# WonderfulToolchain/psxavenc

Hardware: AMD Instinct MI355X
Metric: bs_v2_320x240_frames_per_sec (higher is better)
Workload: dtype int32

## Files before the change

psxavenc_amd/csrc/mdec_kernels.hip:

```cpp

#include <hip/hip_runtime.h>
#include <stdint.h>
#include <type_traits>
#include <stdlib.h>
#include <string.h>

#include "bs_vlc_lut.h"
#include "mdec_search.h"
#include "psxhip_internal.h"
#include "wave_ops.h"

namespace {

constexpr int kWavesSmall = 12, kOccSmall = 6;
constexpr int kWavesLarge = 16, kOccLarge = 4;
constexpr int kTileStride = 72;
constexpr int kZStride = 64;
constexpr int kPilotMax = 4;
constexpr int kMaxTiles = 16;
constexpr uint32_t kNoMb = 0xFFFFu;
constexpr uint32_t kRetryEmpty = 0xFFFFFFFFu, kRetryAbandoned = 0xFFFFFFFEu;
constexpr int kQueueWord = 64;
constexpr int kStartedWord = 96;
constexpr int kLeaveWord = 8;
// ... 926 lines not shown
            phi = *(const uint2*)(frame + o_hi);
        };
        auto fetch = [&](int fx, int fy) { fetch_at((uint32_t)fy * (uint32_t)(8 * W), (uint32_t)fx * 16u); };
        auto mb_bytes = [&](const uint4& ts, uint32_t& b_lo, uint32_t& b_hi) {
            b_lo = __builtin_amdgcn_perm(plo.y, plo.x, ts.x);
            b_hi = __builtin_amdgcn_perm(phi.y, phi.x, ts.y);
        };
        auto fetch_behind = [&](uint32_t row, uint32_t col, uint32_t& b_lo, uint32_t& b_hi) {
            asm volatile("" : "+v"(b_lo), "+v"(b_hi));
            const uint4 tp = L.tab_pix[lane];
            uint32_t o_lo = tp.x + (row << tp.z) + col;
            asm volatile("" : "+v"(o_lo) : "v"(b_lo), "v"(b_hi));
            const uint32_t o_hi = o_lo + tp.y;
            plo = *(const uint2*)(frame + o_lo);
            phi = *(const uint2*)(frame + o_hi);
        };
        auto dct_mb = [&](const uint4& ts, uint32_t b_lo, uint32_t b_hi) {
            int d[8];
            u32x16 ck;
            asm volatile("s_load_dwordx16 %0, %1, %2" : "=s"(ck) : "s"(__builtin_amdgcn_kernarg_segment_ptr()), "n"(offsetof(FrameJob, col_k)));
            {
                fdct8_rows_mfma(b_lo, b_hi, make_uint2(ts.z, ts.w), d);
                const int n = lane & 31;
                int16_t* t0 = tileT + (n >> 3) * kTileStride + (n & 7) + (lane >> 5) * 32;
                store_row_outputs(t0, d);
                if (n < 16) store_row_outputs(t0 + 4 * kTileStride, d + 4);
            }
            wave_sync();
            if (lane < 48) {
                uint4 q;
                asm volatile("ds_read2_b64 %0, %2 offset1:1\n\ts_waitcnt lgkmcnt(0)"
                             : "=v"(q), "+s"(ck) : "v"((uint32_t)(uintptr_t)&tileT[blk * kTileStride + r8 * 8]) : "memory");
                fdct8_col_acc_k(q.x, q.y, __builtin_amdgcn_alignbit(q.w, q.w, 16), __builtin_amdgcn_alignbit(q.z, q.z, 16), ck, d);
                if (r8 == 0) d[0] = CODEC == 0 ? (int)((uint32_t)quant_dc(d[0] >> 17) << 17) : 0;
                uint4 o;
                o.x = pack_sh17(d[1], d[0]);
                o.y = pack_sh17(d[3], d[2]);
                o.z = pack_sh17(d[5], d[4]);
                o.w = pack_sh17(d[7], d[6]);
                *(uint4*)&tileZ[lane * 8] = o;
            }
            wave_sync();
        };

        if (tid == 0) {
            int hint = L.scalars[S_HINT];
            int hint_budget = L.scalars[S_HINT_BUDGET];
            bool local = hint >= 1 && L.scalars[S_HINT_FRAME] == f - 1;
            if (hint < 1) {
                const int sh = L.scalars[S_SHARED_HINT];
                hint = sh & 0xFF;
                hint_budget = sh >> 8;
            }
            const int retry_scale = L.scalars[S_RETRY];
            if (retry_scale > 0) {
                hint = retry_scale;
                hint_budget = max_size;
                local = true;
            }
            const bool hint_ok = hint >= 1 && hint <= 63 && hint_budget == max_size;
            const int dts = L.scalars[S_DISTRUST];
            const int rp = L.scalars[S_REPILOT];
            const int trust_mode = PSX_JOB_INT(trust_mode);
            const bool distrust = trust_mode == 0 ? ((dts & 1) != 0 || (dts >> 8) >= 2) : trust_mode == 2;
            const bool trust_hint = hint_ok && (local || !distrust) && rp == 0;
            L.scalars[S_ABORTS_LEFT] = rp ? 1 : 2;
            L.scalars[S_FOREIGN] = hint_ok && !local ? hint : 0;
// ... 18 lines not shown
                st.fail = (uint64_t)(uint32_t)z | ((uint64_t)(uint32_t)in_loop(0) << 32);
                st.fs[0] = st.fs[1] = st.fb[0] = st.fb[1] = z;
                st.gs[0] = st.gs[1] = st.gb[0] = st.gb[1] = z;
            }
        };
        unsigned long long trace = 0;
        int n_pass = 0, first_abort = 0, guess0 = 0;
        int guess;
        MdecSearch* srch = (MdecSearch*)&L.scalars[S_SEARCH];
        group_sync(1);
        if (L.scalars[S_PILOT_GUESS] == 0) {
        float cfp[kPilotPerWave][6];
#pragma unroll
        for (int i = 0; i < kPilotPerWave; i++) {
            const int pi = wid + i * kWavesPerGroup;
            if (pi < n_pilot) {
                const unsigned u = (unsigned)(2 * pi + 1);
                const int p_fy = (int)((u * (unsigned)ny) / (unsigned)(2 * n_pilot));
                const int p_fx = (int)((((u * 40503u) >> 1) & 0xFFFFu) * (unsigned)nx >> 16);
                fetch(n_pilot == nmb ? pi % nx : p_fx, n_pilot == nmb ? pi / nx : p_fy);
                {
                    const uint4 ts = L.tab_sel[lane];
                    uint32_t b_lo, b_hi;
                    mb_bytes(ts, b_lo, b_hi);
                    dct_mb(ts, b_lo, b_hi);
                }
#pragma unroll
                for (int b = 0; b < 6; b++) cf[b] = lane == 0 ? 0.0f : (float)(int)tileZ[b * kZStride + lc.zsrc];
                wave_sync();
            }
#pragma unroll
            for (int b = 0; b < 6; b++) cfp[i][b] = pi < n_pilot ? cf[b] : 0.0f;
        }
        if (tid == 0) {
            L.scalars[S_PILOTED] = 1;
            const int h0 = L.scalars[S_PILOT_HI];
            MdecSearch st;
            search_reset(st);
            *srch = st;
            const MdecPilot pl = mdec_pilot_next(st, h0, limit_bits, fixed_bits, 0);
            L.scalars[S_PILOT_N] = pl.n;
            L.scalars[S_PILOT_SCALE0 + 0] = pl.s[0];
            L.scalars[S_PILOT_SCALE0 + 1] = pl.s[1];
            L.scalars[S_PILOT_SCALE0 + 2] = pl.s[2];
            L.scalars[S_PILOT_LO] = in_loop(0);
        }
        for (;;) {
            group_sync(1);
            const int np = L.scalars[S_PILOT_N];
            if (np == 0) break;
            if (wid < n_pilot) {
                for (int j = 0; j < np; j++) {
                    const int s = L.scalars[S_PILOT_SCALE0 + j];
                    const QuantK k = make_quant(lc.quant, s);
                    int acc = 0;
#pragma unroll
                    for (int i = 0; i < kPilotPerWave; i++)
                        if (i < pilot_rounds) acc += count_mb(cfp[i], k, lc, L.ac_len16) & 0xFF;
                    const int t = wave::reduce_add(acc);
                    if (lane == 0) atomicAdd(&L.scalars[S_PILOT_BITS0 + j], t);
                }
            }
            group_sync(1);
            if (tid == 0) {
                MdecSearch st = *srch;
                for (int j = 0; j < np; j++) {
                    const int s = L.scalars[S_PILOT_SCALE0 + j];
                    const int est = (int)((long long)L.scalars[S_PILOT_BITS0 + j] * nmb / n_pilot) + fixed_bits;
                    mdec_search_note(st, s, est, est, limit_bits);
                    L.scalars[S_PILOT_BITS0 + j] = 0;
                }
                *srch = st;
                const int round = L.scalars[S_PILOT_LO] + 1;
                const MdecPilot pl = mdec_pilot_next(st, L.scalars[S_PILOT_HI], limit_bits, fixed_bits, round);
                L.scalars[S_PILOT_N] = pl.n;
                L.scalars[S_PILOT_LO] = round;
                L.scalars[S_PILOT_SCALE0 + 0] = pl.s[0];
                L.scalars[S_PILOT_SCALE0 + 1] = pl.s[1];
                L.scalars[S_PILOT_SCALE0 + 2] = pl.s[2];
                if (pl.n == 0) L.scalars[S_PILOT_GUESS] = pl.guess;
            }
        }
        }
        guess = L.scalars[S_PILOT_GUESS];
        if (STATS) { guess0 = carry_pass ? carry_guess0 : guess; if (carry_pass) first_abort = carry_abort; }
        mark(2);

        if (tid == 0) {
            L.scalars[S_NEXT_DRAW] = (int)next_draw;
            MdecSearch st;
            search_reset(st);
            MdecPass np;
            if (limit_bits < fixed_bits || bad_budget) {
                np.done = 1; np.count_scale = 0; np.emit_scale = 0;
            } else {
                np = mdec_search_next(st, guess, limit_bits, fixed_bits);
            }
            *srch = st;
            L.scalars[S_PASS_COUNT] = np.count_scale;
            L.scalars[S_PASS_EMIT] = np.emit_scale;
            L.scalars[S_DONE] = np.done;
            L.scalars[S_RESULT] = st.best;
            L.scalars[S_MB_NEXT] = 2 * kWavesPerGroup;
        }
        group_sync(1);

        while (!L.scalars[S_DONE]) {
            const int count_scale = L.scalars[S_PASS_COUNT], emit_scale = L.scalars[S_PASS_EMIT];
            n_pass++;
            if (STATS && n_pass <= 4) trace |= (unsigned long long)(emit_scale ? emit_scale : count_scale | 0x40) << (24 + 8 * n_pass);
            if (emit_scale && n_pass > 1) {
                for (int i = tid; i < job.stg_words; i += kThreads) L.stg[i] = 0u;
                if (tid == 0) L.scalars[S_STG_NEXT] = 0;
                group_sync(5);
            }
            typedef const char __attribute__((address_space(4))) * OrderBytes;
            typedef const uint32_t __attribute__((address_space(4))) * OrderPtr;
            const OrderBytes order_b = (OrderBytes)(uintptr_t)job.order;
            const int n_tickets = job.trips * kWavesPerGroup;
            auto order_at = [&](int t) -> uint2 {
                const uint32_t byte = min((uint32_t)t, (uint32_t)n_tickets) * 8u;
                const OrderPtr e = (OrderPtr)(order_b + byte);
                return make_uint2(e[0], e[1]);
            };
            int cur_t = wid, nxt_t = wid + kWavesPerGroup;
            uint2 cur_o = order_at(cur_t);
            uint2 nxt_o = order_at(nxt_t);
            fetch_at(cur_o.x & 0x7FFFFFFFu, cur_o.y & 0xFFFFu);
            const QuantK kc = make_quant(lc.quant, count_scale ? count_scale : 1);
            const QuantK ke = make_quant(lc.quant, emit_scale ? emit_scale : 1);
            int acc_cnt = 0;
            int acc_edef = 0;
            int n_codes = 0;
            int emit_bits = 0, mb_done = 0;
            int prev_len = 0;
            const uint32_t thr_low = (uint32_t)((lc.quant * (count_scale ? count_scale : 1) + 1) >> 1);
            const uint32_t thr_emit = (uint32_t)((lc.quant * (emit_scale ? emit_scale : 1) + 1) >> 1);
            const uint32_t thr_list = count_scale ? thr_low : thr_emit;
            const uint32_t low_off = thr_list - 1u, low_span = lane == 0 ? 0u : 2u * thr_list - 1u;
            const uint32_t emit_off = thr_emit - 1u, emit_span = lane == 0 ? 0u : 2u * thr_emit - 1u;
            auto flush = [&]() {
                if (count_scale) {
                    const int tf = wave::reduce_add(acc_cnt & 0xFFFF), td = wave::reduce_add((int)((unsigned)acc_cnt >> 16));
                    if (lane == 0) { atomicAdd(&L.scalars[S_CNT_F], tf); atomicAdd(&L.scalars[S_CNT_D], td); }
                    acc_cnt = 0;
                }
                if (emit_scale) {
                    const int td = wave::reduce_add(acc_edef), tc = n_codes;
                    if (lane == 0) {
                        atomicAdd(&L.scalars[S_EMIT_BITS], emit_bits);
                        atomicAdd(&L.scalars[S_EMIT_D], td);
                        atomicAdd(&L.scalars[S_NNZ], tc - 6 * mb_done);
                    }
                    acc_edef = 0; n_codes = 0; emit_bits = 0;
                }
                if (lane == 0) atomicAdd(&L.scalars[S_CK_DONE], mb_done);
                mb_done = 0;
            };
            const int check_t = (job.trips >= 8 && L.scalars[S_ABORTS_LEFT] > 0) ? (job.trips >> 2) * kWavesPerGroup : n_tickets;
            bool aborted = false, checked = false;

            for (int it = 0; cur_t < n_tickets; it++) {
                if (!checked && cur_t >= check_t) {
                    checked = true;
                    flush();
                    int arrived = 0;
                    if (lane == 0) arrived = atomicAdd(&L.scalars[S_CK_WAVES], 1);
                    const bool judge = __builtin_amdgcn_readfirstlane(arrived) == kWavesPerGroup - 1;
                    unsigned ck_s1 = 0, ck_sq = 0;
                    bool records_ok = false;
                    if (judge && emit_scale) records_ok = __hip_atomic_load(&L.scalars[S_STG_NEXT], __ATOMIC_RELAXED, __HIP_MEMORY_SCOPE_WORKGROUP) <= job.stg_words;
                    if (records_ok) {
                        for (int t = lane; t < check_t; t += 64) {
                            const OrderPtr oe = (OrderPtr)(order_b + (uint32_t)t * 8u);
                            if ((int)oe[0] < 0) {
                                const unsigned x = *(const uint32_t*)((const char*)L.rec + (oe[1] >> 16)) >> 18;
                                ck_s1 += x;
                                ck_sq += x * x;
                            }
                        }
                        ck_s1 = (unsigned)wave::reduce_add((int)ck_s1);
                        ck_sq = (unsigned)wave::reduce_add((int)ck_sq);
                    }
                    if (judge && lane == 0) {
                        const int done = L.scalars[S_CK_DONE];
                        long long pa = 0, pb = 0;
                        if (count_scale) pa = (long long)L.scalars[S_CNT_F] * nmb / done + fixed_bits;
                        if (emit_scale) pb = (long long)L.scalars[S_EMIT_BITS] * nmb / done + 10;
                        int margin = (limit_bits - fixed_bits) / 50;
                        if (emit_scale && records_ok && done > 1 && done < nmb) {
                            const float n = (float)done, mean = (float)ck_s1 / n;
                            float var = (float)ck_sq / n - mean * mean;
                            var = var > 0.0f ? var : 0.0f;
                            const float se = 4.0f * __builtin_sqrtf(var * n * (1.0f - n / (float)nmb)) * ((float)nmb / n);
                            margin = (int)(se * kCkMargin * 0.001f);
                        }
                        int g = mdec_search_checkpoint_bits(*srch, count_scale, (int)pa, emit_scale, (int)pb, limit_bits, fixed_bits, margin);
                        {
                            const int cur = emit_scale ? emit_scale : count_scale + 1, far = cur > 8 ? cur >> 2 : 2;
                            if (g && L.scalars[S_PILOTED] && (g - cur >= far || cur - g >= far)) {
                                const bool too_low = emit_scale && pb > (long long)limit_bits + 4 * margin;
                                const bool too_high = count_scale && pa <= (long long)limit_bits - 4 * margin;
                                if (!too_low && !too_high) g = 0;
                            }
                        }
                        if (g) {
                            L.scalars[S_ABORT] = g | (n_pass << 8);
                            L.scalars[S_ABORTS_LEFT] = L.scalars[S_ABORTS_LEFT] - 1;
                            atomicMax(&L.scalars[S_MB_NEXT], 0x40000000);
                        }
                    }
                }
                if (WAVES == kWavesSmall) {
                    asm volatile("s_bitcmp1_b32 %0, %1\n\ts_cbranch_scc1 1f\n\ts_setprio 0\n\ts_branch 2f\n1:\ts_setprio 1\n2:" : : "s"(prio_bits4), "s"(it) : "scc");
                }
                int drawn = 0;
                if (lane == 0) drawn = atomicAdd(&L.scalars[S_MB_NEXT], 1);
                const bool valid = (int)cur_o.x < 0;
                const uint32_t rec_byte = cur_o.y >> 16;
                const int mbe = (int)(rec_byte >> 2);
                {
                    const uint4 ts = L.tab_sel[lane];
                    uint32_t b_lo, b_hi;
                    mb_bytes(ts, b_lo, b_hi);
                    fetch_behind(nxt_o.x & 0x7FFFFFFFu, nxt_o.y & 0xFFFFu, b_lo, b_hi);
                    if (valid) dct_mb(ts, b_lo, b_hi);
                }
                cur_t = nxt_t;
                cur_o = nxt_o;
                nxt_t = __builtin_amdgcn_readfirstlane(drawn);
                nxt_o = order_at(nxt_t);
                if (!valid) continue;
                mb_done++;

                int ci[6];
#pragma unroll
                for (int b = 0; b < 6; b++) ci[b] = (int)tileZ[b * kZStride + lc.zsrc];
                wave_sync();

                if (!emit_scale) {
                    float cff[6];
#pragma unroll
                    for (int b = 0; b < 6; b++) cff[b] = lane == 0 ? 0.0f : (float)ci[b];
                    const int a = count_mb(cff, kc, lc, L.ac_len16);
                    acc_cnt += (a & 0xFF) | ((a >> 8) << 16);
                    continue;
                }
                constexpr std::true_type yes{};
                constexpr std::false_type no{};
                auto emit_mb = [&](auto cs_tag) {
                    constexpr bool cs = decltype(cs_tag)::value;
                    auto build_list = [&](uint32_t off, uint32_t span) -> int {
                        const uint32_t cb0 = (uint32_t)(uintptr_t)clist;
                        uint32_t cb = cb0, t, e, tag, n;
                        unsigned long long sv;
#define PSX_LIST_BLOCK(CI)                                                \
                            "v_add_u32 %[t], %[off], %[" CI "]\n\t"                \
                            "v_cmp_ge_u32 vcc, %[t], %[span]\n\t"                  \
                            "v_and_or_b32 %[e], %[" CI "], %[m17], %[tag]\n\t"      \
                            "s_and_saveexec_b64 %[sv], vcc\n\t"                    \
                            "v_mbcnt_lo_u32_b32 %[t], vcc_lo, 0\n\t"               \
                            "v_mbcnt_hi_u32_b32 %[t], vcc_hi, %[t]\n\t"            \
                            "v_lshl_add_u32 %[t], %[t], 2, %[cb]\n\t"              \
                            "ds_write_b32 %[t], %[e]\n\t"                          \
                            "s_mov_b64 exec, %[sv]\n\t"                            \
                            "s_bcnt1_i32_b64 %[n], vcc\n\t"                        \
                            "s_lshl2_add_u32 %[cb], %[n], %[cb]\n\t"
                        asm volatile("v_lshlrev_b32 %[tag], 17, %[lane]\n\t"
                                     PSX_LIST_BLOCK("c0") PSX_LIST_BLOCK("c1") PSX_LIST_BLOCK("c2")
                                     PSX_LIST_BLOCK("c3") PSX_LIST_BLOCK("c4") PSX_LIST_BLOCK("c5")
                                     : [cb] "+s"(cb), [t] "=&v"(t), [e] "=&v"(e), [tag] "=&v"(tag), [n] "=&s"(n), [sv] "=&s"(sv)
                                     : [off] "v"(off), [span] "v"(span), [m17] "s"(0x1FFFFu), [lane] "v"(lane),
                                       [c0] "v"(ci[0]), [c1] "v"(ci[1]), [c2] "v"(ci[2]), [c3] "v"(ci[3]), [c4] "v"(ci[4]), [c5] "v"(ci[5])
                                     : "vcc", "scc", "memory");
#undef PSX_LIST_BLOCK
                        asm("s_sub_u32 %0, %1, %2\n\ts_lshr_b32 %0, %0, 2" : "=s"(n) : "s"(cb), "s"(cb0) : "scc");
                        return (int)n;
                    };
                    bool dense = false;
                    int count = 0;
                    if (cs && prev_len > 128) {
                        int n_low = 0;
#pragma unroll
                        for (int b = 0; b < 6; b++) n_low += (int)__builtin_popcountll(wave::ballot((uint32_t)ci[b] + low_off >= low_span));
                        prev_len = n_low;
                        dense = n_low > 128;
                    }
                    if (!dense) {
                        count = build_list(low_off, low_span);
                        if (cs) {
                            prev_len = count;
                            dense = count > 128;
                        }
                    }
                    if (dense) {
                        float cff[6];
#pragma unroll
                        for (int b = 0; b < 6; b++) cff[b] = lane == 0 ? 0.0f : (float)ci[b];
                        const int a = count_mb(cff, kc, lc, L.ac_len16);
                        acc_cnt += (a & 0xFF) | ((a >> 8) << 16);
                        wave_sync();
                        count = build_list(emit_off, emit_span);
                    }
                    wave_sync();

                    int kcarry_a = 0, kcarry_b = 0, bcarry = 0;
                    auto chunk = [&](auto low_tag, auto count_tag, auto single_tag, int base, int& len, uint32_t& code, int& deficit, int& cnt16, int& ncodes) {
                        constexpr bool low = decltype(low_tag)::value, do_count = decltype(count_tag)::value, single = decltype(single_tag)::value;
                        const int i = base + lane;
                        const bool live = i < count;
                        uint32_t e = clist[i];
                        e = live ? e : (63u << 17);
                        const int k = (int)__builtin_amdgcn_ubfe(e, 17, 6);
                        const uint32_t negbit = __builtin_amdgcn_ubfe(e, 16, 1);
                        const bool is_dc = k == 0;
                        const uint64_t dcm = CODEC == 0 ? 0ull : wave::ballot(k == 0);
                        const bool is_ac = live && !is_dc;
                        float magf;
                        asm("v_cvt_f32_i32_sdwa %0, sext(%1) dst_sel:DWORD dst_unused:UNUSED_PAD src0_sel:WORD_0" : "=v"(magf) : "v"(e));
                        cnt16 = 0;
                        int kprev;
                        bool is_last;
                        QuantK ek;
                        ek.inv = __builtin_bit_cast(float, __builtin_amdgcn_ds_bpermute(k << 2, __builtin_bit_cast(int, ke.inv)));
                        ek.bias = __builtin_fmaf(0.25f, ek.inv, 0.5f);
                        uint32_t kbase = (uint32_t)(uintptr_t)(clist + 64);
                        if (low) asm volatile("" : "+s"(kbase));
                        if (low) {
                            const int ka = __builtin_amdgcn_update_dpp(kcarry_a, k, 0x138, 0xF, 0xF, false);
                            if (do_count) {
                                QuantK ck;
                                ck.inv = __builtin_bit_cast(float, __builtin_amdgcn_ds_bpermute(k << 2, __builtin_bit_cast(int, kc.inv)));
                                ck.bias = __builtin_fmaf(0.25f, ck.inv, 0.5f);
                                const int qa = quant_mag(magf, ck);
                                uint32_t lw = L.ac_len16[lut_index(is_ac ? qa : 0, is_ac ? k - ka - 1 : 0)];
                                asm("" : "+v"(lw));
                                cnt16 = (int)__builtin_amdgcn_perm(0u, lw, 0x0C010C00u);
                            }
                            if (!single) kcarry_a = __builtin_amdgcn_readlane(k, 63);
                        }
                        const int q = quant_mag(magf, ek);
                        if (low) {
                            static_assert(single || !low, "a list at the count scale is one chunk");
                            const uint64_t sm = ballot_ne0(q) | ballot_eq0(k);
                            ncodes = (int)__builtin_popcountll(sm);
                            const uint32_t kslot = kbase + 4u * (uint32_t)wave::popc_below(sm);
                            unsigned long long sv;
                            asm volatile("s_and_saveexec_b64 %0, %1\n\tds_write_b32 %2, %3\n\ts_mov_b64 exec, %0"
                                         : "=&s"(sv) : "s"(sm), "v"(kslot), "v"(k) : "memory");
                            typedef const uint32_t __attribute__((address_space(3))) * LdsWord;
                            kprev = (int)*(LdsWord)(uintptr_t)(kslot - 4u);
                            int last = 63 - __builtin_clzll(sm);
                            asm("" : "+s"(last));
                            is_last = lane == last;
                        } else {
                            is_last = i == count - 1;
                            kprev = __builtin_amdgcn_update_dpp(kcarry_b, k, 0x138, 0xF, 0xF, false);
                            if (!single) kcarry_b = __builtin_amdgcn_readlane(k, 63);
                            ncodes = count - base < 64 ? count - base : 64;
                        }
                        const int run_raw = k + ~kprev;
                        const unsigned qrow = (unsigned)q > (unsigned)(BS_LUT_MAX_LEVEL + 1) ? (unsigned)(BS_LUT_MAX_LEVEL + 1) : (unsigned)q;
                        const int li = (int)__umul24(qrow, (unsigned)BS_LUT_W) + run_raw;
                        const uint32_t entry = L.ac_code[is_ac ? li : 0];
                        len = (int)(entry >> 24);
                        code = (entry & 0x1FFFFu) | negbit;
                        if (ballot_eq<BS_ESCAPE_BITS>(len)) {
                            asm volatile("; escape codes");
                            const int lim = 510 + 2 * (int)negbit;
                            const int qc = q > lim ? lim : q;
                            const int sl = (qc ^ -(int)negbit) + (int)negbit;
                            const uint32_t esc = (1u << 16) | ((uint32_t)run_raw << 10) | ((uint32_t)sl & 0x3FFu);
                            code = len == BS_ESCAPE_BITS ? esc : code;
                        }
                        deficit = (int)((entry >> BS_LUT_DEFICIT_SHIFT) & 0xFu);
                        if (CODEC == 0) {
                            if (is_dc) {
                                const uint32_t eob = i != 0 ? 2u << 10 : 0u;
                                code = (e & 0x3FFu) | eob;
                                len = i != 0 ? 12 : 10;
                            }
                        } else {
                            const uint64_t dcmask = dcm;
                            if (is_dc) {
                                const int bi = bcarry + wave::popc_below(dcmask);
                                dc_code<CODEC>((int)L.dcv[mbe * 6 + bi], bi >= 2, L.dc_plen, L.dc_prefix, len, code);
                                if (bi > 0) {
                                    code |= 2u << len;
                                    len += 2;
                                }
                            }
                            if (!single) bcarry += (int)__builtin_popcountll(dcmask);
                        }
                        {
                            const int add = is_last ? 2 : 0;
                            code = (code << add) | (uint32_t)add;
                            len += add;
                        }
                    };
                    bool have_room = true;
                    auto stage_alloc = [&](uint32_t mb_bits) -> uint32_t {
                        const int ndw = (int)((mb_bits + 31u) >> 5);
                        int off = 0;
                        if (lane == 0) {
                            off = atomicAdd(&L.scalars[S_STG_NEXT], ndw);
                            *(uint32_t*)((char*)L.rec + rec_byte) = (uint32_t)off | (mb_bits << 16);
                        }
                        off = __builtin_amdgcn_readfirstlane(off);
                        have_room = off + ndw <= job.stg_words;
                        emit_bits += (int)mb_bits;
                        return (uint32_t)off;
                    };
                    auto put_codes = [&](uint32_t base_dw, uint32_t bit, int len, uint32_t code) {
                        if (have_room) {
                            if (len) put_bits_lds(L.stg, base_dw, bit, len, code);
                        }
                    };
                    bool low = cs && !dense;
                    if (low && count > 64) {
                        int sc = 0, kcarry = 0;
                        for (int base = 0; base < count; base += 64) {
                            const int i = base + lane;
                            const bool live = i < count;
                            uint32_t e = clist[i];
                            e = live ? e : (63u << 17);
                            const int k = (int)__builtin_amdgcn_ubfe(e, 17, 6);
                            const bool is_dc = k == 0;
                            const bool is_ac = live && !is_dc;
                            float magf;
                            asm("v_cvt_f32_i32_sdwa %0, sext(%1) dst_sel:DWORD dst_unused:UNUSED_PAD src0_sel:WORD_0" : "=v"(magf) : "v"(e));
                            QuantK ck, ek;
                            ck.inv = __builtin_bit_cast(float, __builtin_amdgcn_ds_bpermute(k << 2, __builtin_bit_cast(int, kc.inv)));
                            ck.bias = __builtin_fmaf(0.25f, ck.inv, 0.5f);
                            ek.inv = __builtin_bit_cast(float, __builtin_amdgcn_ds_bpermute(k << 2, __builtin_bit_cast(int, ke.inv)));
                            ek.bias = __builtin_fmaf(0.25f, ek.inv, 0.5f);
                            const int ka = __builtin_amdgcn_update_dpp(kcarry, k, 0x138, 0xF, 0xF, false);
                            kcarry = __builtin_amdgcn_readlane(k, 63);
                            const int qa = quant_mag(magf, ck);
                            uint32_t lw = L.ac_len16[lut_index(is_ac ? qa : 0, is_ac ? k - ka - 1 : 0)];
                            asm("" : "+v"(lw));
                            acc_cnt += (int)__builtin_amdgcn_perm(0u, lw, 0x0C010C00u);
                            const int qe = quant_mag(magf, ek);
                            const uint64_t sm = ballot_ne0(qe) | ballot_eq0(k);
                            const uint32_t slot = (uint32_t)(uintptr_t)(clist + sc + wave::popc_below(sm));
                            unsigned long long sv;
                            asm volatile("s_and_saveexec_b64 %0, %1\n\tds_write_b32 %2, %3\n\ts_mov_b64 exec, %0"
                                         : "=&s"(sv) : "s"(sm), "v"(slot), "v"(e) : "memory");
                            sc += (int)__builtin_popcountll(sm);
                        }
                        wave_sync();
                        count = sc;
                        low = false;
                    }
                    if (count <= 64) {
                        int len, deficit, cnt16, nc;
                        uint32_t code;
                        if (low) chunk(yes, yes, yes, 0, len, code, deficit, cnt16, nc);
                        else chunk(no, no, yes, 0, len, code, deficit, cnt16, nc);
                        const int incl = wave::inclusive_scan_add(len);
                        const uint32_t base_dw = stage_alloc((uint32_t)__builtin_amdgcn_readlane(incl, 63));
                        put_codes(base_dw, (uint32_t)(incl - len), len, code);
                        acc_edef += deficit;
                        acc_cnt += cnt16;
                        n_codes += nc;
                    } else {
                        int lsum = 0;
                        for (int base = 0; base < count; base += 64) {
                            int len, deficit, cnt16, nc;
                            uint32_t code;
                            chunk(no, no, no, base, len, code, deficit, cnt16, nc);
                            lsum += len;
                        }
                        const uint32_t base_dw = stage_alloc((uint32_t)wave::reduce_add(lsum));
                        uint32_t pos = 0;
                        kcarry_a = 0;
                        kcarry_b = 0;
                        bcarry = 0;
                        for (int base = 0; base < count; base += 64) {
                            int len, deficit, cnt16, nc;
                            uint32_t code;
                            chunk(no, no, no, base, len, code, deficit, cnt16, nc);
                            const int incl = wave::inclusive_scan_add(len);
                            put_codes(base_dw, pos + (uint32_t)(incl - len), len, code);
                            pos += (uint32_t)__builtin_amdgcn_readlane(incl, 63);
                            acc_edef += deficit;
                            n_codes += nc;
                        }
                    }
                    wave_sync();
                };
                if (count_scale) emit_mb(yes);
                else emit_mb(no);
            }
            if (WAVES == kWavesSmall) __builtin_amdgcn_s_setprio(2);
            flush();
            group_sync(3);
            const int verdict = L.scalars[S_ABORT];
            aborted = (verdict >> 8) == n_pass;
            if (STATS && tid == 0 && aborted && !first_abort) first_abort = verdict & 0xFF;
            if (STATS && aborted && n_pass <= 4) trace |= 0x80ull << (24 + 8 * n_pass);
            if (scan_early && wid == 1 && emit_scale && !aborted) scan_offsets(lane);
            if (tid == 0) {
                MdecSearch st = *srch;
                auto hand_on = [&](const MdecPass& np) -> bool {
                    if (!job.retry || np.done || !np.emit_scale || L.scalars[S_RETRY] != 0 ||
                        (L.scalars[S_RUN_LEFT] == 0 && (unsigned)L.scalars[S_NEXT_DRAW] >= fresh_draws())) return false;
                    const unsigned slot = (unsigned)(atomicAdd(queue_state(job), 1ull << kQueueReservedShift) >> kQueueReservedShift) & kQueueMask;
                    if (atomicExch(&retry_slots(job)[slot], (unsigned)f | ((unsigned)np.emit_scale << 24)) == kRetryAbandoned) {
                        atomicExch(&retry_slots(job)[slot], (unsigned)in_loop((int)kRetryEmpty));
                        return false;
                    }
                    L.scalars[S_DEFER] = 1;
                    L.scalars[S_DONE] = 1;
                    int old_hint = L.scalars[S_HINT_BUDGET] == max_size ? L.scalars[S_HINT] : 0;
                    if (old_hint < 1 && (L.scalars[S_SHARED_HINT] >> 8) == max_size) old_hint = L.scalars[S_SHARED_HINT] & 0xFF;
                    L.scalars[S_HINT] = old_hint < 1 || L.scalars[S_PUSHED] ? np.emit_scale : old_hint;
                    L.scalars[S_HINT_BUDGET] = max_size;
                    L.scalars[S_HINT_FRAME] = in_loop(-2);
                    L.scalars[S_PUSHED] = 1;
                    if (L.scalars[S_FOREIGN] && !L.scalars[S_PILOTED]) {
                        L.scalars[S_F_TRIED] = L.scalars[S_F_TRIED] + 1;
                        L.scalars[S_F_WRONG] = L.scalars[S_F_WRONG] + 1;
                        L.scalars[S_DISTRUST] = L.scalars[S_DISTRUST] + 0x100;
                    }
                    return true;
// ... 512 lines not shown
```

psxavenc_amd/csrc/psxhip_internal.h:

```cpp
#pragma once
#include <hip/hip_runtime.h>
#include <stddef.h>
#include <stdint.h>

#include "../../include/psxav_hip.h"

#define PSXHIP_MDEC_KERNEL_REV "mdec-k3.8"
#define PSXHIP_ADPCM_KERNEL_REV "adpcm-k5.4"

#ifdef __cplusplus
extern "C" {
#endif

typedef struct {
	const psxhip_mdec_batch_t *batches;
	int n_batches;
	size_t frame_stride;
	int width, height, codec;
	int n_frames;
	int n_tickets;
	int uniform_max_size;
	size_t out_stride;
	int out_words;
	int out_tile;
	int max_frame_size;
	int stg_words;
	int grid;
	int large;
	void *stream;
	unsigned int *d_ticket;
	unsigned int *d_hint;
	unsigned int *d_retry;
	int retry_cap;
	int retry_patience;
	unsigned long long *d_stats;
	int trust_mode;
	const uint32_t *d_order;
} psxhip_mdec_launch_t;

typedef struct {
// ... 122 lines not shown
```

Measured before the change: 8.678 million.

## Batch sparse macroblocks' codes across iterations into one wave-wide emit pass

Macroblocks with few coefficients are now staged in a pending per-lane buffer, and several of them are encoded together in one 64-lane VLC emit pass. The block index is packed into the DC word so block and record identity survive the batching. The aim is to use more lanes in the bitstream emission, which sat mostly idle for sparse macroblocks. The change also reshapes the main ticket loop and moves the bit and nnz counters to per-emit atomics. It adds complexity and more LDS atomics, and it risks ordering or record bugs around checkpoints.

```diff
diff --git a/psxavenc_amd/csrc/mdec_kernels.hip b/psxavenc_amd/csrc/mdec_kernels.hip
--- a/psxavenc_amd/csrc/mdec_kernels.hip
+++ b/psxavenc_amd/csrc/mdec_kernels.hip
@@ -982,7 +982,7 @@
                 asm volatile("ds_read2_b64 %0, %2 offset1:1\n\ts_waitcnt lgkmcnt(0)"
                              : "=v"(q), "+s"(ck) : "v"((uint32_t)(uintptr_t)&tileT[blk * kTileStride + r8 * 8]) : "memory");
                 fdct8_col_acc_k(q.x, q.y, __builtin_amdgcn_alignbit(q.w, q.w, 16), __builtin_amdgcn_alignbit(q.z, q.z, 16), ck, d);
-                if (r8 == 0) d[0] = CODEC == 0 ? (int)((uint32_t)quant_dc(d[0] >> 17) << 17) : 0;
+                if (r8 == 0) d[0] = (CODEC == 0 ? (quant_dc(d[0] >> 17) & 0x3FF) | (blk << 10) : blk) << 17;
                 uint4 o;
                 o.x = pack_sh17(d[1], d[0]);
                 o.y = pack_sh17(d[3], d[2]);
@@ -1067,7 +1067,7 @@
 #pragma unroll
             for (int b = 0; b < 6; b++) cfp[i][b] = pi < n_pilot ? cf[b] : 0.0f;
         }
-        if (tid == 0) {
+        if (in_loop(tid) == 0) {
             L.scalars[S_PILOTED] = 1;
             const int h0 = L.scalars[S_PILOT_HI];
             MdecSearch st;
@@ -1097,7 +1097,7 @@
                 }
             }
             group_sync(1);
-            if (tid == 0) {
+            if (in_loop(tid) == 0) {
                 MdecSearch st = *srch;
                 for (int j = 0; j < np; j++) {
                     const int s = L.scalars[S_PILOT_SCALE0 + j];
@@ -1121,7 +1121,7 @@
         if (STATS) { guess0 = carry_pass ? carry_guess0 : guess; if (carry_pass) first_abort = carry_abort; }
         mark(2);
 
-        if (tid == 0) {
+        if (in_loop(tid) == 0) {
             L.scalars[S_NEXT_DRAW] = (int)next_draw;
             MdecSearch st;
             search_reset(st);
@@ -1166,8 +1166,7 @@
             const QuantK ke = make_quant(lc.quant, emit_scale ? emit_scale : 1);
             int acc_cnt = 0;
             int acc_edef = 0;
-            int n_codes = 0;
-            int emit_bits = 0, mb_done = 0;
+            int mb_done = 0;
             int prev_len = 0;
             const uint32_t thr_low = (uint32_t)((lc.quant * (count_scale ? count_scale : 1) + 1) >> 1);
             const uint32_t thr_emit = (uint32_t)((lc.quant * (emit_scale ? emit_scale : 1) + 1) >> 1);
@@ -1181,13 +1180,9 @@
                     acc_cnt = 0;
                 }
                 if (emit_scale) {
-                    const int td = wave::reduce_add(acc_edef), tc = n_codes;
-                    if (lane == 0) {
-                        atomicAdd(&L.scalars[S_EMIT_BITS], emit_bits);
-                        atomicAdd(&L.scalars[S_EMIT_D], td);
-                        atomicAdd(&L.scalars[S_NNZ], tc - 6 * mb_done);
-                    }
-                    acc_edef = 0; n_codes = 0; emit_bits = 0;
+                    const int td = wave::reduce_add(acc_edef);
+                    if (lane == 0) atomicAdd(&L.scalars[S_EMIT_D], td);
+                    acc_edef = 0;
                 }
                 if (lane == 0) atomicAdd(&L.scalars[S_CK_DONE], mb_done);
                 mb_done = 0;
@@ -1195,153 +1190,291 @@
             const int check_t = (job.trips >= 8 && L.scalars[S_ABORTS_LEFT] > 0) ? (job.trips >> 2) * kWavesPerGroup : n_tickets;
             bool aborted = false, checked = false;
 
-            for (int it = 0; cur_t < n_tickets; it++) {
-                if (!checked && cur_t >= check_t) {
-                    checked = true;
-                    flush();
-                    int arrived = 0;
-                    if (lane == 0) arrived = atomicAdd(&L.scalars[S_CK_WAVES], 1);
-                    const bool judge = __builtin_amdgcn_readfirstlane(arrived) == kWavesPerGroup - 1;
-                    unsigned ck_s1 = 0, ck_sq = 0;
-                    bool records_ok = false;
-                    if (judge && emit_scale) records_ok = __hip_atomic_load(&L.scalars[S_STG_NEXT], __ATOMIC_RELAXED, __HIP_MEMORY_SCOPE_WORKGROUP) <= job.stg_words;
-                    if (records_ok) {
-                        for (int t = lane; t < check_t; t += 64) {
-                            const OrderPtr oe = (OrderPtr)(order_b + (uint32_t)t * 8u);
-                            if ((int)oe[0] < 0) {
-                                const unsigned x = *(const uint32_t*)((const char*)L.rec + (oe[1] >> 16)) >> 18;
-                                ck_s1 += x;
-                                ck_sq += x * x;
+            int pend = 0;
+            uint32_t pendv = 0;
+            constexpr int kBiShift = CODEC == 0 ? 10 : 0;
+            auto emit_pending = [&]() {
+                const int n = pend & 0xFF, m = pend >> 8;
+                pend = 0;
+                const bool live = lane < n;
+                const uint32_t e = live ? pendv : (63u << 17);
+                const int k = (int)__builtin_amdgcn_ubfe(e, 17, 6);
+                const int kprev = __builtin_amdgcn_update_dpp(0, k, 0x138, 0xF, 0xF, false);
+                const uint32_t negbit = __builtin_amdgcn_ubfe(e, 16, 1);
+                const bool is_dc = k == 0;
+                const bool is_ac = live && !is_dc;
+                const bool first = (e & ((63u << 17) | (7u << kBiShift))) == 0u;
+                const uint64_t firstm = wave::ballot(first);
+                const uint64_t lastm = (firstm >> 1) | (1ull << (n - 1));
+                const int mbe_l = (int)(__builtin_amdgcn_ubfe(e, 13, 4) | ((e >> 23) << 4));
+                const int q = (int)(e & 0xFFFFu);
+                const int run_raw = k + ~kprev;
+                const unsigned qrow = (unsigned)q > (unsigned)(BS_LUT_MAX_LEVEL + 1) ? (unsigned)(BS_LUT_MAX_LEVEL + 1) : (unsigned)q;
+                const int li = (int)__umul24(qrow, (unsigned)BS_LUT_W) + run_raw;
+                const uint32_t entry = L.ac_code[is_ac ? li : 0];
+                int len = (int)(entry >> 24);
+                uint32_t code = (entry & 0x1FFFFu) | negbit;
+                if (ballot_eq<BS_ESCAPE_BITS>(len)) {
+                    asm volatile("; escape codes");
+                    const int lim = 510 + 2 * (int)negbit;
+                    const int qc = q > lim ? lim : q;
+                    const int sl = (qc ^ -(int)negbit) + (int)negbit;
+                    const uint32_t esc = (1u << 16) | ((uint32_t)run_raw << 10) | ((uint32_t)sl & 0x3FFu);
+                    code = len == BS_ESCAPE_BITS ? esc : code;
+                }
+                acc_edef += (int)((entry >> BS_LUT_DEFICIT_SHIFT) & 0xFu);
+                if (CODEC == 0) {
+                    if (is_dc) {
+                        code = (e & 0x3FFu) | (first ? 0u : 2u << 10);
+                        len = first ? 10 : 12;
+                    }
+                } else {
+                    if (is_dc) {
+                        const int bi = (int)(e & 7u);
+                        dc_code<CODEC>((int)L.dcv[mbe_l * 6 + bi], bi >= 2, L.dc_plen, L.dc_prefix, len, code);
+                        if (!first) {
+                            code |= 2u << len;
+                            len += 2;
+                        }
+                    }
+                }
+                {
+                    int add;
+                    asm("v_cndmask_b32_e64 %0, 0, 2, %1" : "=v"(add) : "s"(lastm));
+                    code = (code << add) | (uint32_t)add;
+                    len += add;
+                }
+                const int incl = wave::inclusive_scan_add(len);
+                uint32_t pos = (uint32_t)(incl - len), piece = 0, done_bits = 0, recv = 0;
+                uint64_t rem = lastm;
+                int fj = 0;
+                while (rem) {
+                    const int lj = (int)__builtin_ctzll(rem);
+                    rem &= rem - 1ull;
+                    const uint32_t upto = (uint32_t)__builtin_amdgcn_readlane(incl, lj);
+                    const uint32_t bits = upto - done_bits;
+                    recv = lane == fj ? (piece >> 5) | (bits << 16) : recv;
+                    const uint32_t next = (piece + bits + 31u) & ~31u;
+                    pos += lane > lj ? next - (piece + bits) : 0u;
+                    piece = next;
+                    done_bits = upto;
+                    fj = lj + 1;
+                }
+                const int ndw = (int)(piece >> 5);
+                int off = 0;
+                if (lane == 0) {
+                    off = atomicAdd(&L.scalars[S_STG_NEXT], ndw);
+                    atomicAdd(&L.scalars[S_EMIT_BITS], (int)done_bits);
+                    atomicAdd(&L.scalars[S_NNZ], n - 6 * m);
+                }
+                off = __builtin_amdgcn_readfirstlane(off);
+                if (first) L.rec[mbe_l] = recv + (uint32_t)off;
+                if (off + ndw <= job.stg_words) {
+                    if (len) put_bits_lds(L.stg, (uint32_t)off, pos, len, code);
+                }
+                if (STATS && lane == 0) {
+                    atomicAdd(&job.stats[PSXHIP_MDEC_STATS_PHASE0 + 14], 1ull);
+                    atomicAdd(&job.stats[PSXHIP_MDEC_STATS_PHASE0 + 15], (unsigned long long)m);
+                }
+            };
+
+            constexpr std::true_type yes{};
+            constexpr std::false_type no{};
+            for (int it = 0;;) {
+                bool have_mb = false, dense = false, defer = false;
+                int count = 0, sc = 65;
+                uint32_t rec_byte = 0;
+                bool emit_now = pend && (cur_t >= n_tickets || (!checked && cur_t >= check_t));
+                if (!emit_now) {
+                if (cur_t >= n_tickets) break;
+                    if (!checked && cur_t >= check_t) {
+                        checked = true;
+                        flush();
+                        int arrived = 0;
+                        if (lane == 0) arrived = atomicAdd(&L.scalars[S_CK_WAVES], 1);
+                        const bool judge = __builtin_amdgcn_readfirstlane(arrived) == kWavesPerGroup - 1;
+                        unsigned ck_s1 = 0, ck_sq = 0;
+                        bool records_ok = false;
+                        if (judge && emit_scale) records_ok = __hip_atomic_load(&L.scalars[S_STG_NEXT], __ATOMIC_RELAXED, __HIP_MEMORY_SCOPE_WORKGROUP) <= job.stg_words;
+                        if (records_ok) {
+                            for (int t = lane; t < check_t; t += 64) {
+                                const OrderPtr oe = (OrderPtr)(order_b + (uint32_t)t * 8u);
+                                if ((int)oe[0] < 0) {
+                                    const unsigned x = *(const uint32_t*)((const char*)L.rec + (oe[1] >> 16)) >> 18;
+                                    ck_s1 += x;
+                                    ck_sq += x * x;
+                                }
+                            }
+                            ck_s1 = (unsigned)wave::reduce_add((int)ck_s1);
+                            ck_sq = (unsigned)wave::reduce_add((int)ck_sq);
+                        }
+                        if (judge && lane == 0) {
+                            const int done = L.scalars[S_CK_DONE];
+                            long long pa = 0, pb = 0;
+                            if (count_scale) pa = (long long)L.scalars[S_CNT_F] * nmb / done + fixed_bits;
+                            if (emit_scale) pb = (long long)L.scalars[S_EMIT_BITS] * nmb / done + 10;
+                            int margin = (limit_bits - fixed_bits) / 50;
+                            if (emit_scale && records_ok && done > 1 && done < nmb) {
+                                const float n = (float)done, mean = (float)ck_s1 / n;
+                                float var = (float)ck_sq / n - mean * mean;
+                                var = var > 0.0f ? var : 0.0f;
+                                const float se = 4.0f * __builtin_sqrtf(var * n * (1.0f - n / (float)nmb)) * ((float)nmb / n);
+                                margin = (int)(se * kCkMargin * 0.001f);
+                            }
+                            int g = mdec_search_checkpoint_bits(*srch, count_scale, (int)pa, emit_scale, (int)pb, limit_bits, fixed_bits, margin);
+                            {
+                                int cur = emit_scale ? emit_scale : count_scale + 1;
+                                    asm volatile("" : "+s"(cur));
+                                    const int far = cur > 8 ? cur >> 2 : 2;
+                                if (g && L.scalars[S_PILOTED] && (g - cur >= far || cur - g >= far)) {
+                                    const bool too_low = emit_scale && pb > (long long)limit_bits + 4 * margin;
+                                    const bool too_high = count_scale && pa <= (long long)limit_bits - 4 * margin;
+                                    if (!too_low && !too_high) g = 0;
+                                }
+                            }
+                            if (g) {
+                                L.scalars[S_ABORT] = g | (n_pass << 8);
+                                L.scalars[S_ABORTS_LEFT] = L.scalars[S_ABORTS_LEFT] - 1;
+                                atomicMax(&L.scalars[S_MB_NEXT], 0x40000000);
                             }
                         }
-                        ck_s1 = (unsigned)wave::reduce_add((int)ck_s1);
-                        ck_sq = (unsigned)wave::reduce_add((int)ck_sq);
-                    }
-                    if (judge && lane == 0) {
-                        const int done = L.scalars[S_CK_DONE];
-                        long long pa = 0, pb = 0;
-                        if (count_scale) pa = (long long)L.scalars[S_CNT_F] * nmb / done + fixed_bits;
-                        if (emit_scale) pb = (long long)L.scalars[S_EMIT_BITS] * nmb / done + 10;
-                        int margin = (limit_bits - fixed_bits) / 50;
-                        if (emit_scale && records_ok && done > 1 && done < nmb) {
-                            const float n = (float)done, mean = (float)ck_s1 / n;
-                            float var = (float)ck_sq / n - mean * mean;
-                            var = var > 0.0f ? var : 0.0f;
-                            const float se = 4.0f * __builtin_sqrtf(var * n * (1.0f - n / (float)nmb)) * ((float)nmb / n);
-                            margin = (int)(se * kCkMargin * 0.001f);
-                        }
-                        int g = mdec_search_checkpoint_bits(*srch, count_scale, (int)pa, emit_scale, (int)pb, limit_bits, fixed_bits, margin);
-                        {
-                            const int cur = emit_scale ? emit_scale : count_scale + 1, far = cur > 8 ? cur >> 2 : 2;
-                            if (g && L.scalars[S_PILOTED] && (g - cur >= far || cur - g >= far)) {
-                                const bool too_low = emit_scale && pb > (long long)limit_bits + 4 * margin;
-                                const bool too_high = count_scale && pa <= (long long)limit_bits - 4 * margin;
-                                if (!too_low && !too_high) g = 0;
-                            }
-                        }
-                        if (g) {
-                            L.scalars[S_ABORT] = g | (n_pass << 8);
-                            L.scalars[S_ABORTS_LEFT] = L.scalars[S_ABORTS_LEFT] - 1;
-                            atomicMax(&L.scalars[S_MB_NEXT], 0x40000000);
-                        }
-                    }
-                }
-                if (WAVES == kWavesSmall) {
-                    asm volatile("s_bitcmp1_b32 %0, %1\n\ts_cbranch_scc1 1f\n\ts_setprio 0\n\ts_branch 2f\n1:\ts_setprio 1\n2:" : : "s"(prio_bits4), "s"(it) : "scc");
-                }
-                int drawn = 0;
-                if (lane == 0) drawn = atomicAdd(&L.scalars[S_MB_NEXT], 1);
-                const bool valid = (int)cur_o.x < 0;
-                const uint32_t rec_byte = cur_o.y >> 16;
-                const int mbe = (int)(rec_byte >> 2);
-                {
-                    const uint4 ts = L.tab_sel[lane];
-                    uint32_t b_lo, b_hi;
-                    mb_bytes(ts, b_lo, b_hi);
-                    fetch_behind(nxt_o.x & 0x7FFFFFFFu, nxt_o.y & 0xFFFFu, b_lo, b_hi);
-                    if (valid) dct_mb(ts, b_lo, b_hi);
-                }
-                cur_t = nxt_t;
-                cur_o = nxt_o;
-                nxt_t = __builtin_amdgcn_readfirstlane(drawn);
-                nxt_o = order_at(nxt_t);
-                if (!valid) continue;
-                mb_done++;
-
-                int ci[6];
+                    }
+                    if (WAVES == kWavesSmall) {
+                        asm volatile("s_bitcmp1_b32 %0, %1\n\ts_cbranch_scc1 1f\n\ts_setprio 0\n\ts_branch 2f\n1:\ts_setprio 1\n2:" : : "s"(prio_bits4), "s"(it) : "scc");
+                    }
+                    it++;
+                    int drawn = 0;
+                    if (lane == 0) drawn = atomicAdd(&L.scalars[S_MB_NEXT], 1);
+                    const bool valid = (int)cur_o.x < 0;
+                    rec_byte = cur_o.y >> 16;
+                    {
+                        const uint4 ts = L.tab_sel[lane];
+                        uint32_t b_lo, b_hi;
+                        mb_bytes(ts, b_lo, b_hi);
+                        fetch_behind(nxt_o.x & 0x7FFFFFFFu, nxt_o.y & 0xFFFFu, b_lo, b_hi);
+                        if (valid) dct_mb(ts, b_lo, b_hi);
+                    }
+                    cur_t = nxt_t;
+                    cur_o = nxt_o;
+                    nxt_t = __builtin_amdgcn_readfirstlane(drawn);
+                    nxt_o = order_at(nxt_t);
+                    if (!valid) continue;
+                    mb_done++;
+
+                    int ci[6];
 #pragma unroll
-                for (int b = 0; b < 6; b++) ci[b] = (int)tileZ[b * kZStride + lc.zsrc];
-                wave_sync();
-
-                if (!emit_scale) {
-                    float cff[6];
-#pragma unroll
-                    for (int b = 0; b < 6; b++) cff[b] = lane == 0 ? 0.0f : (float)ci[b];
-                    const int a = count_mb(cff, kc, lc, L.ac_len16);
-                    acc_cnt += (a & 0xFF) | ((a >> 8) << 16);
-                    continue;
-                }
-                constexpr std::true_type yes{};
-                constexpr std::false_type no{};
-                auto emit_mb = [&](auto cs_tag) {
-                    constexpr bool cs = decltype(cs_tag)::value;
-                    auto build_list = [&](uint32_t off, uint32_t span) -> int {
-                        const uint32_t cb0 = (uint32_t)(uintptr_t)clist;
-                        uint32_t cb = cb0, t, e, tag, n;
-                        unsigned long long sv;
-#define PSX_LIST_BLOCK(CI)                                                \
-                            "v_add_u32 %[t], %[off], %[" CI "]\n\t"                \
-                            "v_cmp_ge_u32 vcc, %[t], %[span]\n\t"                  \
-                            "v_and_or_b32 %[e], %[" CI "], %[m17], %[tag]\n\t"      \
-                            "s_and_saveexec_b64 %[sv], vcc\n\t"                    \
-                            "v_mbcnt_lo_u32_b32 %[t], vcc_lo, 0\n\t"               \
-                            "v_mbcnt_hi_u32_b32 %[t], vcc_hi, %[t]\n\t"            \
-                            "v_lshl_add_u32 %[t], %[t], 2, %[cb]\n\t"              \
-                            "ds_write_b32 %[t], %[e]\n\t"                          \
-                            "s_mov_b64 exec, %[sv]\n\t"                            \
-                            "s_bcnt1_i32_b64 %[n], vcc\n\t"                        \
-                            "s_lshl2_add_u32 %[cb], %[n], %[cb]\n\t"
-                        asm volatile("v_lshlrev_b32 %[tag], 17, %[lane]\n\t"
-                                     PSX_LIST_BLOCK("c0") PSX_LIST_BLOCK("c1") PSX_LIST_BLOCK("c2")
-                                     PSX_LIST_BLOCK("c3") PSX_LIST_BLOCK("c4") PSX_LIST_BLOCK("c5")
-                                     : [cb] "+s"(cb), [t] "=&v"(t), [e] "=&v"(e), [tag] "=&v"(tag), [n] "=&s"(n), [sv] "=&s"(sv)
-                                     : [off] "v"(off), [span] "v"(span), [m17] "s"(0x1FFFFu), [lane] "v"(lane),
-                                       [c0] "v"(ci[0]), [c1] "v"(ci[1]), [c2] "v"(ci[2]), [c3] "v"(ci[3]), [c4] "v"(ci[4]), [c5] "v"(ci[5])
-                                     : "vcc", "scc", "memory");
-#undef PSX_LIST_BLOCK
-                        asm("s_sub_u32 %0, %1, %2\n\ts_lshr_b32 %0, %0, 2" : "=s"(n) : "s"(cb), "s"(cb0) : "scc");
-                        return (int)n;
-                    };
-                    bool dense = false;
-                    int count = 0;
-                    if (cs && prev_len > 128) {
-                        int n_low = 0;
-#pragma unroll
-                        for (int b = 0; b < 6; b++) n_low += (int)__builtin_popcountll(wave::ballot((uint32_t)ci[b] + low_off >= low_span));
-                        prev_len = n_low;
-                        dense = n_low > 128;
-                    }
-                    if (!dense) {
-                        count = build_list(low_off, low_span);
-                        if (cs) {
-                            prev_len = count;
-                            dense = count > 128;
-                        }
-                    }
-                    if (dense) {
+                    for (int b = 0; b < 6; b++) ci[b] = (int)tileZ[b * kZStride + lc.zsrc];
+                    wave_sync();
+
+                    if (!emit_scale) {
                         float cff[6];
 #pragma unroll
                         for (int b = 0; b < 6; b++) cff[b] = lane == 0 ? 0.0f : (float)ci[b];
                         const int a = count_mb(cff, kc, lc, L.ac_len16);
                         acc_cnt += (a & 0xFF) | ((a >> 8) << 16);
+                        continue;
+                    }
+                    auto mb_list = [&](auto cs_tag) {
+                        constexpr bool cs = decltype(cs_tag)::value;
+                        auto build_list = [&](uint32_t off, uint32_t span) -> int {
+                            const uint32_t cb0 = (uint32_t)(uintptr_t)clist;
+                            uint32_t cb = cb0, t, e, tag, n;
+                            unsigned long long sv;
+#define PSX_LIST_BLOCK(CI)                                                \
+                                "v_add_u32 %[t], %[off], %[" CI "]\n\t"                \
+                                "v_cmp_ge_u32 vcc, %[t], %[span]\n\t"                  \
+                                "v_and_or_b32 %[e], %[" CI "], %[m17], %[tag]\n\t"      \
+                                "s_and_saveexec_b64 %[sv], vcc\n\t"                    \
+                                "v_mbcnt_lo_u32_b32 %[t], vcc_lo, 0\n\t"               \
+                                "v_mbcnt_hi_u32_b32 %[t], vcc_hi, %[t]\n\t"            \
+                                "v_lshl_add_u32 %[t], %[t], 2, %[cb]\n\t"              \
+                                "ds_write_b32 %[t], %[e]\n\t"                          \
+                                "s_mov_b64 exec, %[sv]\n\t"                            \
+                                "s_bcnt1_i32_b64 %[n], vcc\n\t"                        \
+                                "s_lshl2_add_u32 %[cb], %[n], %[cb]\n\t"
+                            asm volatile("v_lshlrev_b32 %[tag], 17, %[lane]\n\t"
+                                         PSX_LIST_BLOCK("c0") PSX_LIST_BLOCK("c1") PSX_LIST_BLOCK("c2")
+                                         PSX_LIST_BLOCK("c3") PSX_LIST_BLOCK("c4") PSX_LIST_BLOCK("c5")
+                                         : [cb] "+s"(cb), [t] "=&v"(t), [e] "=&v"(e), [tag] "=&v"(tag), [n] "=&s"(n), [sv] "=&s"(sv)
+                                         : [off] "v"(off), [span] "v"(span), [m17] "s"(0x1FFFFu), [lane] "v"(lane),
+                                           [c0] "v"(ci[0]), [c1] "v"(ci[1]), [c2] "v"(ci[2]), [c3] "v"(ci[3]), [c4] "v"(ci[4]), [c5] "v"(ci[5])
+                                         : "vcc", "scc", "memory");
+#undef PSX_LIST_BLOCK
+                            asm("s_sub_u32 %0, %1, %2\n\ts_lshr_b32 %0, %0, 2" : "=s"(n) : "s"(cb), "s"(cb0) : "scc");
+                            return (int)n;
+                        };
+                        if (cs && prev_len > 128) {
+                            int n_low = 0;
+#pragma unroll
+                            for (int b = 0; b < 6; b++) n_low += (int)__builtin_popcountll(wave::ballot((uint32_t)ci[b] + low_off >= low_span));
+                            prev_len = n_low;
+                            dense = n_low > 128;
+                        }
+                        if (!dense) {
+                            count = build_list(low_off, low_span);
+                            if (cs) {
+                                prev_len = count;
+                                dense = count > 128;
+                            }
+                        }
+                        if (dense) {
+                            float cff[6];
+#pragma unroll
+                            for (int b = 0; b < 6; b++) cff[b] = lane == 0 ? 0.0f : (float)ci[b];
+                            const int a = count_mb(cff, kc, lc, L.ac_len16);
+                            acc_cnt += (a & 0xFF) | ((a >> 8) << 16);
+                            wave_sync();
+                            count = build_list(emit_off, emit_span);
+                        }
                         wave_sync();
-                        count = build_list(emit_off, emit_span);
-                    }
-                    wave_sync();
-
-                    int kcarry_a = 0, kcarry_b = 0, bcarry = 0;
-                    auto chunk = [&](auto low_tag, auto count_tag, auto single_tag, int base, int& len, uint32_t& code, int& deficit, int& cnt16, int& ncodes) {
-                        constexpr bool low = decltype(low_tag)::value, do_count = decltype(count_tag)::value, single = decltype(single_tag)::value;
+
+                        defer = !dense && count <= 64;
+                        if (defer) {
+                            const bool live = lane < count;
+                            uint32_t e = clist[lane];
+                            e = live ? e : (63u << 17);
+                            const int k = (int)__builtin_amdgcn_ubfe(e, 17, 6);
+                            const bool is_dc = k == 0;
+                            float magf;
+                            asm("v_cvt_f32_i32_sdwa %0, sext(%1) dst_sel:DWORD dst_unused:UNUSED_PAD src0_sel:WORD_0" : "=v"(magf) : "v"(e));
+                            QuantK ek;
+                            ek.inv = __builtin_bit_cast(float, __builtin_amdgcn_ds_bpermute(k << 2, __builtin_bit_cast(int, ke.inv)));
+                            ek.bias = __builtin_fmaf(0.25f, ek.inv, 0.5f);
+                            if (cs) {
+                                const bool is_ac = live && !is_dc;
+                                QuantK ck;
+                                ck.inv = __builtin_bit_cast(float, __builtin_amdgcn_ds_bpermute(k << 2, __builtin_bit_cast(int, kc.inv)));
+                                ck.bias = __builtin_fmaf(0.25f, ck.inv, 0.5f);
+                                const int ka = __builtin_amdgcn_update_dpp(0, k, 0x138, 0xF, 0xF, false);
+                                const int qa = quant_mag(magf, ck);
+                                uint32_t lw = L.ac_len16[lut_index(is_ac ? qa : 0, is_ac ? k - ka - 1 : 0)];
+                                asm("" : "+v"(lw));
+                                acc_cnt += (int)__builtin_amdgcn_perm(0u, lw, 0x0C010C00u);
+                            }
+                            const int qe = quant_mag(magf, ek);
+                            const uint64_t sm = ballot_ne0(qe) | ballot_eq0(k);
+                            sc = (int)__builtin_popcountll(sm);
+                            const uint32_t mbe = rec_byte >> 2, tag = ((mbe & 0xFu) << 13) | ((mbe >> 4) << 23);
+                            const uint32_t lvl = (e & 0x7F0000u) | (uint32_t)qe, dcs = (e & 0x1FFFu) | tag;
+                            e = is_dc ? dcs : lvl;
+                            const uint32_t slot = (uint32_t)(uintptr_t)(clist + wave::popc_below(sm));
+                            unsigned long long sv;
+                            asm volatile("s_and_saveexec_b64 %0, %1\n\tds_write_b32 %2, %3\n\ts_mov_b64 exec, %0"
+                                         : "=&s"(sv) : "s"(sm), "v"(slot), "v"(e) : "memory");
+                        }
+                    };
+                    if (count_scale) mb_list(yes);
+                    else mb_list(no);
+                    have_mb = true;
+                emit_now = pend && ((pend & 0xFF) + sc > 64 || pend >= 4 << 8);
+                }
+                if (emit_now) emit_pending();
+                if (!have_mb) continue;
+                auto mb_codes = [&](auto cs_tag) {
+                    constexpr bool cs = decltype(cs_tag)::value;
+                    int kcarry_b = 0;
+                    auto chunk = [&](auto single_tag, int base, int& len, uint32_t& code, int& deficit, int& ncodes) {
+                        constexpr bool single = decltype(single_tag)::value;
                         const int i = base + lane;
                         const bool live = i < count;
                         uint32_t e = clist[i];
@@ -1349,51 +1482,17 @@
                         const int k = (int)__builtin_amdgcn_ubfe(e, 17, 6);
                         const uint32_t negbit = __builtin_amdgcn_ubfe(e, 16, 1);
                         const bool is_dc = k == 0;
-                        const uint64_t dcm = CODEC == 0 ? 0ull : wave::ballot(k == 0);
                         const bool is_ac = live && !is_dc;
                         float magf;
                         asm("v_cvt_f32_i32_sdwa %0, sext(%1) dst_sel:DWORD dst_unused:UNUSED_PAD src0_sel:WORD_0" : "=v"(magf) : "v"(e));
-                        cnt16 = 0;
-                        int kprev;
-                        bool is_last;
                         QuantK ek;
                         ek.inv = __builtin_bit_cast(float, __builtin_amdgcn_ds_bpermute(k << 2, __builtin_bit_cast(int, ke.inv)));
                         ek.bias = __builtin_fmaf(0.25f, ek.inv, 0.5f);
-                        uint32_t kbase = (uint32_t)(uintptr_t)(clist + 64);
-                        if (low) asm volatile("" : "+s"(kbase));
-                        if (low) {
-                            const int ka = __builtin_amdgcn_update_dpp(kcarry_a, k, 0x138, 0xF, 0xF, false);
-                            if (do_count) {
-                                QuantK ck;
-                                ck.inv = __builtin_bit_cast(float, __builtin_amdgcn_ds_bpermute(k << 2, __builtin_bit_cast(int, kc.inv)));
-                                ck.bias = __builtin_fmaf(0.25f, ck.inv, 0.5f);
-                                const int qa = quant_mag(magf, ck);
-                                uint32_t lw = L.ac_len16[lut_index(is_ac ? qa : 0, is_ac ? k - ka - 1 : 0)];
-                                asm("" : "+v"(lw));
-                                cnt16 = (int)__builtin_amdgcn_perm(0u, lw, 0x0C010C00u);
-                            }
-                            if (!single) kcarry_a = __builtin_amdgcn_readlane(k, 63);
-                        }
                         const int q = quant_mag(magf, ek);
-                        if (low) {
-                            static_assert(single || !low, "a list at the count scale is one chunk");
-                            const uint64_t sm = ballot_ne0(q) | ballot_eq0(k);
-                            ncodes = (int)__builtin_popcountll(sm);
-                            const uint32_t kslot = kbase + 4u * (uint32_t)wave::popc_below(sm);
-                            unsigned long long sv;
-                            asm volatile("s_and_saveexec_b64 %0, %1\n\tds_write_b32 %2, %3\n\ts_mov_b64 exec, %0"
-                                         : "=&s"(sv) : "s"(sm), "v"(kslot), "v"(k) : "memory");
-                            typedef const uint32_t __attribute__((address_space(3))) * LdsWord;
-                            kprev = (int)*(LdsWord)(uintptr_t)(kslot - 4u);
-                            int last = 63 - __builtin_clzll(sm);
-                            asm("" : "+s"(last));
-                            is_last = lane == last;
-                        } else {
-                            is_last = i == count - 1;
-                            kprev = __builtin_amdgcn_update_dpp(kcarry_b, k, 0x138, 0xF, 0xF, false);
-                            if (!single) kcarry_b = __builtin_amdgcn_readlane(k, 63);
-                            ncodes = count - base < 64 ? count - base : 64;
-                        }
+                        const bool is_last = i == count - 1;
+                        const int kprev = __builtin_amdgcn_update_dpp(kcarry_b, k, 0x138, 0xF, 0xF, false);
+                        if (!single) kcarry_b = __builtin_amdgcn_readlane(k, 63);
+                        ncodes = count - base < 64 ? count - base : 64;
                         const int run_raw = k + ~kprev;
                         const unsigned qrow = (unsigned)q > (unsigned)(BS_LUT_MAX_LEVEL + 1) ? (unsigned)(BS_LUT_MAX_LEVEL + 1) : (unsigned)q;
                         const int li = (int)__umul24(qrow, (unsigned)BS_LUT_W) + run_raw;
@@ -1416,16 +1515,14 @@
                                 len = i != 0 ? 12 : 10;
                             }
                         } else {
-                            const uint64_t dcmask = dcm;
                             if (is_dc) {
-                                const int bi = bcarry + wave::popc_below(dcmask);
-                                dc_code<CODEC>((int)L.dcv[mbe * 6 + bi], bi >= 2, L.dc_plen, L.dc_prefix, len, code);
+                                const int bi = (int)(e & 7u);
+                                dc_code<CODEC>((int)L.dcv[(rec_byte >> 2) * 6 + bi], bi >= 2, L.dc_plen, L.dc_prefix, len, code);
                                 if (bi > 0) {
                                     code |= 2u << len;
                                     len += 2;
                                 }
                             }
-                            if (!single) bcarry += (int)__builtin_popcountll(dcmask);
                         }
                         {
                             const int add = is_last ? 2 : 0;
@@ -1440,10 +1537,11 @@
                         if (lane == 0) {
                             off = atomicAdd(&L.scalars[S_STG_NEXT], ndw);
                             *(uint32_t*)((char*)L.rec + rec_byte) = (uint32_t)off | (mb_bits << 16);
+                            atomicAdd(&L.scalars[S_EMIT_BITS], (int)mb_bits);
+                            atomicAdd(&L.scalars[S_NNZ], count - 6);
                         }
                         off = __builtin_amdgcn_readfirstlane(off);
                         have_room = off + ndw <= job.stg_words;
-                        emit_bits += (int)mb_bits;
                         return (uint32_t)off;
                     };
                     auto put_codes = [&](uint32_t base_dw, uint32_t bit, int len, uint32_t code) {
@@ -1451,8 +1549,15 @@
                             if (len) put_bits_lds(L.stg, base_dw, bit, len, code);
                         }
                     };
-                    bool low = cs && !dense;
-                    if (low && count > 64) {
+                    if (defer) {
+                        const int at = lane - (pend & 0xFF);
+                        wave_sync();
+                        if ((unsigned)at < (unsigned)sc) pendv = clist[at];
+                        pend += sc + 0x100;
+                        wave_sync();
+                        return;
+                    }
+                    if (cs && !dense) {
                         int sc = 0, kcarry = 0;
                         for (int base = 0; base < count; base += 64) {
                             const int i = base + lane;
@@ -1485,47 +1590,44 @@
                         }
                         wave_sync();
                         count = sc;
-                        low = false;
+                    }
+                    if (STATS && lane == 0) {
+                        atomicAdd(&job.stats[PSXHIP_MDEC_STATS_PHASE0 + 14], (unsigned long long)((count + 63) >> 6));
+                        atomicAdd(&job.stats[PSXHIP_MDEC_STATS_PHASE0 + 15], 1ull);
                     }
                     if (count <= 64) {
-                        int len, deficit, cnt16, nc;
+                        int len, deficit, nc;
                         uint32_t code;
-                        if (low) chunk(yes, yes, yes, 0, len, code, deficit, cnt16, nc);
-                        else chunk(no, no, yes, 0, len, code, deficit, cnt16, nc);
+                        chunk(yes, 0, len, code, deficit, nc);
                         const int incl = wave::inclusive_scan_add(len);
                         const uint32_t base_dw = stage_alloc((uint32_t)__builtin_amdgcn_readlane(incl, 63));
                         put_codes(base_dw, (uint32_t)(incl - len), len, code);
                         acc_edef += deficit;
-                        acc_cnt += cnt16;
-                        n_codes += nc;
                     } else {
                         int lsum = 0;
                         for (int base = 0; base < count; base += 64) {
-                            int len, deficit, cnt16, nc;
+                            int len, deficit, nc;
                             uint32_t code;
-                            chunk(no, no, no, base, len, code, deficit, cnt16, nc);
+                            chunk(no, base, len, code, deficit, nc);
                             lsum += len;
                         }
                         const uint32_t base_dw = stage_alloc((uint32_t)wave::reduce_add(lsum));
                         uint32_t pos = 0;
-                        kcarry_a = 0;
                         kcarry_b = 0;
-                        bcarry = 0;
                         for (int base = 0; base < count; base += 64) {
-                            int len, deficit, cnt16, nc;
+                            int len, deficit, nc;
                             uint32_t code;
-                            chunk(no, no, no, base, len, code, deficit, cnt16, nc);
+                            chunk(no, base, len, code, deficit, nc);
                             const int incl = wave::inclusive_scan_add(len);
                             put_codes(base_dw, pos + (uint32_t)(incl - len), len, code);
                             pos += (uint32_t)__builtin_amdgcn_readlane(incl, 63);
                             acc_edef += deficit;
-                            n_codes += nc;
                         }
                     }
                     wave_sync();
                 };
-                if (count_scale) emit_mb(yes);
-                else emit_mb(no);
+                if (count_scale) mb_codes(yes);
+                else mb_codes(no);
             }
             if (WAVES == kWavesSmall) __builtin_amdgcn_s_setprio(2);
             flush();
diff --git a/psxavenc_amd/csrc/psxhip_internal.h b/psxavenc_amd/csrc/psxhip_internal.h
--- a/psxavenc_amd/csrc/psxhip_internal.h
+++ b/psxavenc_amd/csrc/psxhip_internal.h
@@ -5,7 +5,7 @@
 
 #include "../../include/psxav_hip.h"
 
-#define PSXHIP_MDEC_KERNEL_REV "mdec-k3.8"
+#define PSXHIP_MDEC_KERNEL_REV "mdec-k3.9"
 #define PSXHIP_ADPCM_KERNEL_REV "adpcm-k5.4"
 
 #ifdef __cplusplus
```

Result: slower. 4.628 million (-46.7%).
